# AndyCGraham/consensusClustR

Measured on AMD Instinct MI355X. Metric: bootstraps/sec (kNN+SNN+co-cluster) at 100k cells, 1/2/4/8 MI355X, higher is better.
Workload: dtype f64

## Files before the change

consensusclustr_amd/csrc/silhouette.hip:

```cpp
#include <math.h>
#include <stdlib.h>
#include <string.h>

#include <algorithm>
#include <vector>

#include "ccg_internal.h"

#define SIL_T 256
#define SIL_CGRP 4
#ifndef SIL_LG
#define SIL_LG 5
#endif

__host__ __device__ __forceinline__ int scale_exp(double bound) {
    if (!(bound > 0.0)) return 52;
    int e = 61 - (ilogb(bound) + 1);
    return e > 52 ? 52 : e;
}

struct SilSegs {
    int nseg;
    const int64_t* off;
    const int32_t* const* lab;
    const int* ts;
    const int* tw;
    double* const* mean;
    int32_t* const* ncl;
    int32_t* const* mns;
};
__device__ __forceinline__ int sil_seg_tile(const int* __restrict__ pre, int nseg, int b) {
    int lo = 0, hi = nseg - 1;
    while (lo < hi) {
        const int mid = (lo + hi + 1) >> 1;
        if (pre[mid] <= b) lo = mid;
        else hi = mid - 1;
    }
    return lo;
}
__device__ __forceinline__ int sil_seg_row(const int64_t* __restrict__ off, int nseg, int64_t r) {
    int lo = 0, hi = nseg - 1;
    while (lo < hi) {
        const int mid = (lo + hi + 1) >> 1;
        if (off[mid] <= r) lo = mid;
        else hi = mid - 1;
    }
    return lo;
}
__device__ __forceinline__ int sil_label(const int32_t* __restrict__ labels, int64_t m, const SilSegs& sg, int q,
                                         int l, int64_t r) {
    if (sg.nseg) {
        const int64_t o = sg.off[q];
        return sg.lab[q][(int64_t)l * (sg.off[q + 1] - o) + (r - o)];
    }
    return labels[(int64_t)l * m + r];
}

#define SIL_MAXABS_GRID 256
#define SIL_MAXABS_T 1024
__global__ __launch_bounds__(SIL_MAXABS_T) void sil_maxabs(const double* __restrict__ x, int64_t tot,
                                                           unsigned* __restrict__ bits) {
    __shared__ unsigned red[SIL_MAXABS_T / 64];
    double mx = 0.0, m1 = 0.0, m2 = 0.0, m3 = 0.0;
    const int64_t stp = (int64_t)gridDim.x * blockDim.x;
    int64_t t = (int64_t)blockIdx.x * blockDim.x + threadIdx.x;
    for (; t + 3 * stp < tot; t += 4 * stp) {
        mx = fmax(mx, fabs(x[t]));
        m1 = fmax(m1, fabs(x[t + stp]));
        m2 = fmax(m2, fabs(x[t + 2 * stp]));
        m3 = fmax(m3, fabs(x[t + 3 * stp]));
    }
    for (; t < tot; t += stp) mx = fmax(mx, fabs(x[t]));
    mx = fmax(fmax(mx, m1), fmax(m2, m3));
    unsigned local = __float_as_uint(nextafterf((float)mx, INFINITY));
    for (int o = 32; o > 0; o >>= 1) local = max(local, (unsigned)__shfl_xor((int)local, o, 64));
    if ((threadIdx.x & 63) == 0) red[threadIdx.x >> 6] = local;
    __syncthreads();
    if (threadIdx.x == 0) {
        unsigned b = red[0];
#pragma unroll
        for (int w = 1; w < SIL_MAXABS_T / 64; ++w) b = max(b, red[w]);
        atomicMax(bits, b);
    }
}

template <int DMAX>
__device__ __forceinline__ void load_row(const double* __restrict__ x, int64_t r, int d,
// ... 9 lines not shown
                                                      int L, int cmax,
                                                      const unsigned* __restrict__ maxabs_bits,
                                                      unsigned long long* __restrict__ gsum,
                                                      unsigned long long* __restrict__ gcnt) {
    extern __shared__ __attribute__((aligned(16))) unsigned char smem[];
    unsigned long long* acc = (unsigned long long*)smem;
    unsigned* cnt = (unsigned*)(acc + (int64_t)(cmax + 1) * d);
    const int64_t r = (int64_t)blockIdx.x * SIL_T + threadIdx.x;
    const bool in = r < m;
    const double maxabs = (double)__uint_as_float(*maxabs_bits);
    const double sc = ldexp(1.0, scale_exp(maxabs * (double)m));
    long long q[DMAX];
#pragma unroll
    for (int k = 0; k < DMAX; ++k) q[k] = (in && k < d) ? __double2ll_rn(x[r * d + k] * sc) : 0ll;
    const int nacc = (cmax + 1) * d;
    const int l1 = min(L, (int)(blockIdx.y + 1) * SIL_LG);
    for (int l = blockIdx.y * SIL_LG; l < l1; ++l) {
        unsigned long long* gs = gsum + (int64_t)l * nacc;
        unsigned long long* gc = gcnt + (int64_t)l * (cmax + 1);
        if (LDS) {
            for (int t = threadIdx.x; t < nacc; t += SIL_T) acc[t] = 0ull;
            for (int t = threadIdx.x; t <= cmax; t += SIL_T) cnt[t] = 0u;
            __syncthreads();
        }
        if (in) {
            const int lab = labels[(int64_t)l * m + r];
            if (lab >= 1 && lab <= cmax) {
#pragma unroll
                for (int k = 0; k < DMAX; ++k)
                    if (k < d) {
                        if (LDS) atomicAdd(&acc[lab * d + k], (unsigned long long)q[k]);
                        else atomicAdd(&gs[(int64_t)lab * d + k], (unsigned long long)q[k]);
                    }
                if (LDS) atomicAdd(&cnt[lab], 1u);
                else atomicAdd(&gc[lab], 1ull);
            }
        }
        if (LDS) {
            __syncthreads();
            for (int t = threadIdx.x; t < nacc; t += SIL_T)
                if (acc[t]) atomicAdd(&gs[t], acc[t]);
            for (int t = threadIdx.x; t <= cmax; t += SIL_T)
                if (cnt[t]) atomicAdd(&gc[t], (unsigned long long)cnt[t]);
            __syncthreads();
        }
    }
}

__device__ __forceinline__ int sil_block_excl_scan(int v, int* sh, int* total) {
    const int t = threadIdx.x, lane = t & 63, wv = t >> 6;
    int x = v;
    for (int o = 1; o < 64; o <<= 1) {
        const int y = __shfl_up(x, o, 64);
        if (lane >= o) x += y;
    }
    if (lane == 63) sh[wv] = x;
    __syncthreads();
    int woff = 0, tot = 0;
    for (int w = 0; w < SIL_T / 64; ++w) {
        if (w < wv) woff += sh[w];
        tot += sh[w];
    }
    __syncthreads();
    *total = tot;
    return woff + x - v;
}

__host__ __device__ inline double sil_s2_bound(double maxabs, int d, int64_t m) {
    return maxabs * maxabs * (double)d * (double)m;
}
template <int DMAX>
__global__ void sil_quant(const double* __restrict__ x, int64_t m, int d, const unsigned* __restrict__ maxabs_bits,
                          long long* __restrict__ q1, long long* __restrict__ q2) {
    const int64_t t = (int64_t)blockIdx.x * blockDim.x + threadIdx.x;
    const int64_t r = t / DMAX;
    if (r >= m) return;
    const int k = (int)(t - r * DMAX);
    const double maxabs = (double)__uint_as_float(*maxabs_bits);
    const double sc = ldexp(1.0, scale_exp(maxabs * (double)m));
    const double v = k < d ? x[r * d + k] : 0.0;
    const long long qv = __double2ll_rn(v * sc);
    q1[t] = qv;
    const double vq = (double)qv / sc;
    double s2 = vq * vq;
#pragma unroll
    for (int o = DMAX / 2; o > 0; o >>= 1) s2 += __shfl_xor(s2, o, 64);
    if (k == 0) q2[r] = __double2ll_rn(s2 * ldexp(1.0, scale_exp(sil_s2_bound(maxabs, d, m))));
}

#define SIL_SB 1024
#define SIL_SP 1024
#ifndef SIL_SGMAX
#define SIL_SGMAX 4
#endif
#define SIL_LDS_CU 163840
#ifndef SIL_LDS_SUMS
#define SIL_LDS_SUMS 81920
#endif
__host__ __device__ inline size_t sil_tile_lds(int d, int cmax, int G) {
    return (size_t)SIL_SP * 4 + (size_t)G * SIL_SP * 8 + (size_t)G * (cmax + 1) * (d + 2) * 8;
}
static inline int sil_sums_G(int d, int cmax) {
    for (int G = SIL_SGMAX; G >= 1; G >>= 1)
        if (sil_tile_lds(d, cmax, G) <= SIL_LDS_SUMS) return G;
    return sil_tile_lds(d, cmax, 1) <= SIL_LDS_CU ? 1 : 0;
}

template <int DMAX, bool SEG>
__global__ __launch_bounds__(SIL_SB) void sil_sums_blk(int64_t m, int d, int ntile, int tpx, int G,
                                                       const int32_t* __restrict__ labels, int L, int cmax,
                                                       const long long* __restrict__ q1,
                                                       const long long* __restrict__ q2,
                                                       unsigned long long* __restrict__ gsum,
                                                       unsigned long long* __restrict__ gsum2,
                                                       unsigned long long* __restrict__ gcnt,
                                                       const int* __restrict__ rep, const int* __restrict__ mult,
                                                       const int* __restrict__ cnt, int64_t mw,
                                                       const int64_t* __restrict__ nrep,
                                                       const int64_t* __restrict__ scan, SilSegs sgs) {
    extern __shared__ __attribute__((aligned(16))) unsigned char smem[];
    int* srow = (int*)smem;
    int* slab = srow + SIL_SP;
    int* swgt = slab + G * SIL_SP;
    unsigned long long* acc = (unsigned long long*)(swgt + G * SIL_SP);
    const int na = (cmax + 1) * (d + 2);
    constexpr int NW = SIL_SB / 64;
    constexpr int RPW = 64 / DMAX;
    constexpr int PPW = SIL_SP / NW;
    const int tid = threadIdx.x, lane = tid & 63, wave = tid >> 6;
    const int k = lane % DMAX, sub = lane / DMAX;
    const int loc = blockIdx.x >> 3;
    const int grp = loc / tpx;
    const int tile = (loc - grp * tpx) * 8 + (blockIdx.x & 7);
    const int l0 = grp * G;
    if (l0 >= L || tile >= ntile) return;
    const int ng = min(G, L - l0);
    int64_t rb, npos;
    int q = 0;
    if constexpr (SEG) {
        q = sil_seg_tile(sgs.ts, sgs.nseg, tile);
        rb = scan[sgs.off[q]] + (int64_t)(tile - sgs.ts[q]) * SIL_SP;
        npos = scan[sgs.off[q + 1]];
    } else {
        rb = (int64_t)tile * SIL_SP;
        npos = rep ? *nrep : m;
    }
    if (rb >= npos) return;
    for (int t = tid; t < ng * na; t += SIL_SB) acc[t] = 0ull;
    for (int p = tid; p < SIL_SP; p += SIL_SB) {
        const int64_t ps = rb + p;
        const bool in = ps < npos;
        const int row = in ? (rep ? rep[ps] : (int)ps) : 0;
        srow[p] = row;
        const int c0 = (in && rep) ? cnt[ps] : 1;
        for (int g = 0; g < G; ++g) {
            int lb = 0, wg = 0;
            if (in && g < ng) {
                const int l = l0 + g;
                if constexpr (SEG) lb = sil_label(labels, m, sgs, q, l, row);
                else lb = labels[(int64_t)l * m + row];
                wg = rep ? c0 - mult[(int64_t)l * mw + ps] : 1;
            }
            const bool ok = lb >= 1 && lb <= cmax && wg > 0;
            slab[g * SIL_SP + p] = ok ? lb : 0;
            swgt[g * SIL_SP + p] = ok ? wg : 0;
        }
    }
    __syncthreads();
    constexpr int SU = 8;
    static_assert((PPW / RPW) % SU == 0, "walk unroll");
    for (int i0 = 0; i0 < PPW / RPW; i0 += SU) {
        int rr[SU];
        long long v[SU], v2[SU];
#pragma unroll
        for (int u = 0; u < SU; ++u) rr[u] = srow[wave * PPW + (i0 + u) * RPW + sub];
#pragma unroll
        for (int u = 0; u < SU; ++u) {
            v[u] = q1[(int64_t)rr[u] * DMAX + k];
            v2[u] = q2[rr[u]];
        }
#pragma unroll
        for (int u = 0; u < SU; ++u) asm volatile("" : "+v"(v[u]), "+v"(v2[u]));
        for (int g = 0; g < ng; ++g) {
            unsigned long long* ag = acc + g * na;
#pragma unroll
            for (int u = 0; u < SU; ++u) {
                const int pl = g * SIL_SP + wave * PPW + (i0 + u) * RPW + sub;
                const int lb = slab[pl];
                if (lb) {
                    const long long w = swgt[pl];
                    if (k < d) atomicAdd(&ag[lb * d + k], (unsigned long long)(w * v[u]));
                    if (k == 0) {
                        atomicAdd(&ag[(cmax + 1) * d + lb], (unsigned long long)(w * v2[u]));
                        atomicAdd(&ag[(cmax + 1) * (d + 1) + lb], (unsigned long long)w);
                    }
                }
            }
        }
    }
    __syncthreads();
    for (int g = 0; g < ng; ++g) {
        const int lv = q * L + l0 + g;
        const unsigned long long* ag = acc + g * na;
        unsigned long long* gs = gsum + (int64_t)lv * (cmax + 1) * d;
        for (int t = tid; t < (cmax + 1) * d; t += SIL_SB) {
            const unsigned long long v = ag[t];
            if (v) atomicAdd(&gs[t], v);
        }
        for (int c = tid; c <= cmax; c += SIL_SB) {
            const unsigned long long n = ag[(cmax + 1) * (d + 1) + c];
            if (n) {
                atomicAdd(&gcnt[(int64_t)lv * (cmax + 1) + c], n);
                atomicAdd(&gsum2[(int64_t)lv * (cmax + 1) + c], ag[(cmax + 1) * d + c]);
            }
        }
    }
}

template <int DMAX>
__global__ void sil_sums_exc(int64_t m, int d, const int32_t* __restrict__ labels, int L, int cmax,
                             const long long* __restrict__ q1, const long long* __restrict__ q2,
                             const unsigned long long* __restrict__ exc, const int* __restrict__ nexc,
                             unsigned long long* __restrict__ gsum, unsigned long long* __restrict__ gsum2,
                             unsigned long long* __restrict__ gcnt, SilSegs sgs) {
    const int ne = *nexc;
    for (int e = blockIdx.x * blockDim.x + threadIdx.x; e < ne; e += gridDim.x * blockDim.x) {
        const int l = (int)(exc[e] >> 32);
        const int64_t r = (int64_t)(exc[e] & 0xffffffffull);
        const int q = sgs.nseg ? sil_seg_row(sgs.off, sgs.nseg, r) : 0;
        const int lab = sil_label(labels, m, sgs, q, l, r);
        if (lab < 1 || lab > cmax) continue;
        const int64_t lv = (int64_t)q * L + l;
        unsigned long long* gs = gsum + (lv * (cmax + 1) + lab) * d;
        for (int k = 0; k < d; ++k) atomicAdd(&gs[k], (unsigned long long)q1[r * DMAX + k]);
        atomicAdd(&gsum2[lv * (cmax + 1) + lab], (unsigned long long)q2[r]);
        atomicAdd(&gcnt[lv * (cmax + 1) + lab], 1ull);
    }
}

template <int DMAX>
__host__ __device__ __forceinline__ int sil_mfma_pos(int k) {
    constexpr int KS = DMAX / 4;
    return (k & 3) * KS + (k >> 2);
}

template <int DMAX>
__global__ __launch_bounds__(SIL_T) void sil_mu(int64_t m, int d, int cmax,
                                                const unsigned* __restrict__ maxabs_bits,
                                                const unsigned long long* __restrict__ gsum,
                                                const unsigned long long* __restrict__ gsum2,
                                                const unsigned long long* __restrict__ gcnt,
                                                int* __restrict__ npres, int* __restrict__ codes,
                                                int* __restrict__ pos, double* __restrict__ mu,
                                                double* __restrict__ muc, double* __restrict__ auxc) {
    __shared__ int sh[SIL_T / 64];
    const int l = blockIdx.x;
    const double maxabs = (double)__uint_as_float(*maxabs_bits);
    const double inv_sc = ldexp(1.0, -scale_exp(maxabs * (double)m));
    const unsigned long long* gs = gsum + (int64_t)l * (cmax + 1) * d;
    const unsigned long long* gc = gcnt + (int64_t)l * (cmax + 1);
    int* pl = pos + (int64_t)l * (cmax + 1);
    int carry = 0;
    for (int c0 = 0; c0 <= cmax; c0 += SIL_T) {
        const int c = c0 + threadIdx.x;
        const bool present = c >= 1 && c <= cmax && gc[c] != 0ull;
        int tot;
        const int ex = carry + sil_block_excl_scan(present ? 1 : 0, sh, &tot);
        if (c <= cmax) pl[c] = present ? ex : -1;
        if (present) codes[(int64_t)l * cmax + ex] = c;
        carry += tot;
    }
    if (threadIdx.x == 0) npres[l] = carry;
    __syncthreads();
    double* ml = mu + (int64_t)l * (cmax + 1) * DMAX;
    double* mcl = muc + (int64_t)l * cmax * DMAX;
    for (int64_t t = threadIdx.x; t < (int64_t)(cmax + 1) * DMAX; t += SIL_T) {
        const int c = (int)(t / DMAX), k = (int)(t - (int64_t)c * DMAX);
        const unsigned long long n = gc[c];
        const double v = (n && k < d) ? ((double)(long long)gs[(int64_t)c * d + k] * inv_sc) / (double)n : 0.0;
        ml[t] = v;
        const int pc = pl[c];
        if (pc >= 0) mcl[(int64_t)pc * DMAX + sil_mfma_pos<DMAX>(k)] = v;
    }
    __syncthreads();
    for (int c = threadIdx.x; c <= cmax; c += SIL_T) {
        const int pc = pl[c];
        if (pc < 0) continue;
        double s = 0.0;
        for (int k = 0; k < d; ++k) s = fma(ml[(int64_t)c * DMAX + k], ml[(int64_t)c * DMAX + k], s);
        auxc[((int64_t)l * cmax + pc) * 2] = s;
        if (gsum2) {
            const double inv_sc2 = ldexp(1.0, -scale_exp(sil_s2_bound(maxabs, d, m)));
            const double n = (double)gc[c];
            const double v = ((double)(long long)gsum2[(int64_t)l * (cmax + 1) + c] * inv_sc2) / n - s;
            const double floor_v = inv_sc2 + 0x1p-50 * s;
            auxc[((int64_t)l * cmax + pc) * 2 + 1] = v > floor_v ? v : 0.0;
        }
    }
}

template <int DMAX, bool LDS>
__global__ __launch_bounds__(SIL_T) void sil_var(const double* __restrict__ x, int64_t m, int d,
                                                 const int32_t* __restrict__ labels, int L, int cmax,
                                                 const unsigned* __restrict__ maxabs_bits,
                                                 const double* __restrict__ mu,
                                                 unsigned long long* __restrict__ gvar) {
    extern __shared__ __attribute__((aligned(16))) unsigned char smem[];
    double* mus = (double*)smem;
    unsigned long long* vacc = (unsigned long long*)(mus + (int64_t)(cmax + 1) * DMAX);
    const int64_t r = (int64_t)blockIdx.x * SIL_T + threadIdx.x;
    const bool in = r < m;
    double xr[DMAX];
    load_row<DMAX>(x, in ? r : 0, d, xr);
    const double maxabs = (double)__uint_as_float(*maxabs_bits);
    const double vb = 4.0 * maxabs * maxabs * (double)d * (double)m;
    const double vsc = ldexp(1.0, scale_exp(vb));
    const int l1 = min(L, (int)(blockIdx.y + 1) * SIL_LG);
    for (int l = blockIdx.y * SIL_LG; l < l1; ++l) {
        const double* ml = mu + (int64_t)l * (cmax + 1) * DMAX;
        unsigned long long* gv = gvar + (int64_t)l * (cmax + 1);
        if (LDS) {
            for (int t = threadIdx.x; t < (cmax + 1) * DMAX; t += SIL_T) mus[t] = ml[t];
// ... 722 lines not shown

#define SIL_MULT_LG 8
__global__ __launch_bounds__(256) void sil_mult_kernel(int64_t m, int L, const int32_t* __restrict__ labels,
                                                       const int64_t* __restrict__ scan,
                                                       const int3* __restrict__ nonrep, int64_t mw,
                                                       int* __restrict__ dis, unsigned long long* __restrict__ exc,
                                                       int* __restrict__ nexc, SilSegs sgs) {
    const int64_t nn = m - scan[m];
    for (int l0 = blockIdx.y * SIL_MULT_LG; l0 < L; l0 += gridDim.y * SIL_MULT_LG)
    for (int64_t j = (int64_t)blockIdx.x * blockDim.x + threadIdx.x; j < nn; j += (int64_t)gridDim.x * blockDim.x) {
        const int3 e = nonrep[j];
        const int r = e.x, rp = e.y;
        const int q = sgs.nseg ? sil_seg_row(sgs.off, sgs.nseg, r) : 0;
        int a[SIL_MULT_LG], b[SIL_MULT_LG];
#pragma unroll
        for (int t = 0; t < SIL_MULT_LG; ++t) {
            a[t] = b[t] = 0;
            if (l0 + t < L) {
                a[t] = sil_label(labels, m, sgs, q, l0 + t, r);
                b[t] = sil_label(labels, m, sgs, q, l0 + t, rp);
            }
        }
#pragma unroll
        for (int t = 0; t < SIL_MULT_LG; ++t) {
            if (a[t] != b[t]) {
                const int l = l0 + t;
                atomicAdd(&dis[(int64_t)l * mw + e.z], 1);
                const int x = atomicAdd(nexc, 1);
                exc[x] = ((unsigned long long)l << 32) | (unsigned long long)r;
            }
        }
    }
}

template <int DMAX>
__global__ void sil_width_exc(const double* __restrict__ x, int64_t m, int d, const int32_t* __restrict__ labels,
                              int L, int cmax, const int* __restrict__ npres, const int* __restrict__ codes,
                              const double* __restrict__ muc, const double* __restrict__ auxc,
                              const unsigned long long* __restrict__ exc, const int* __restrict__ nexc, int nbw,
                              unsigned long long* __restrict__ wsum, unsigned long long* __restrict__ wcnt,
                              SilSegs sgs) {
    const int ne = *nexc;
    for (int e = blockIdx.x * blockDim.x + threadIdx.x; e < ne; e += gridDim.x * blockDim.x) {
    const int l = (int)(exc[e] >> 32);
    const int64_t r = (int64_t)(exc[e] & 0xffffffffull);
    const int q = sgs.nseg ? sil_seg_row(sgs.off, sgs.nseg, r) : 0;
    const int lab = sil_label(labels, m, sgs, q, l, r);
    const int64_t lv = (int64_t)q * L + l;
    double xr[DMAX];
#pragma unroll
    for (int k = 0; k < DMAX; ++k) xr[k] = k < d ? x[r * d + k] : 0.0;
    const int np = npres[lv];
    double self = INFINITY, oth = INFINITY;
    for (int p = 0; p < np; ++p) {
        const double* mp = muc + (lv * cmax + p) * DMAX;
        double s2 = fmax(auxc[2 * (lv * cmax + p) + 1], 0.0);
#pragma unroll
        for (int k = 0; k < DMAX; ++k) {
            const double t = xr[k] - mp[sil_mfma_pos<DMAX>(k)];
            s2 = fma(t, t, s2);
        }
        if (codes[lv * cmax + p] == lab) self = s2;
        else oth = fmin(oth, s2);
    }
    long long wq = 0;
    unsigned wn = 0;
    sil_row_width(self, oth, true, np, ldexp(1.0, scale_exp((double)m)), nullptr, wq, wn);
    if (wn) {
        atomicAdd(&wsum[lv * nbw], (unsigned long long)wq);
        atomicAdd(&wcnt[lv * nbw], 1ull);
    }
    }
}

static int sil_tile_T(int d, int cmax) {
    return sil_sums_G(d, cmax) ? SIL_SP : 0;
}

template <int DMAX>
static void sil_launch(const double* x, int64_t m, int d, const int32_t* labels, int L, int cmax,
                       unsigned* maxabs, unsigned long long* gsum, unsigned long long* gsum2, unsigned long long* gcnt,
                       unsigned long long* gvar, unsigned long long* wsum, unsigned long long* wcnt,
                       int* npres, int* codes, int* pos, double* mu, double* muc, double* auxc, void* q,
                       unsigned char* img, double* out_width, int nbw, hipStream_t st, const int* rep = nullptr,
                       const int* mult = nullptr, const int* cnt = nullptr, int64_t mw = 0,
                       const unsigned long long* exc = nullptr, const int* nexc = nullptr,
                       const int64_t* nrep = nullptr, const int64_t* scan = nullptr, SilSegs sgs = SilSegs{},
                       int ts_tiles = 0, int tw_tiles = 0) {
    const bool seg = sgs.nseg > 0;
    const int Lv = seg ? sgs.nseg * L : L;
    const int T = q ? sil_tile_T(d, cmax) : 0;
    if (T) {
        long long* q1 = (long long*)q;
        long long* q2 = q1 + m * DMAX;
        sil_quant<DMAX><<<(unsigned)ccg_cdiv(m * DMAX, 256), 256, 0, st>>>(x, m, d, maxabs, q1, q2);
        const int ntile = (int)(seg ? ts_tiles : ccg_cdiv(m, T));
        const int tpx = (int)ccg_cdiv(ntile, 8);
        const int G = sil_sums_G(d, cmax);
        const unsigned gb = (unsigned)(8 * (int64_t)tpx * ccg_cdiv(L, G));
        const size_t lds = sil_tile_lds(d, cmax, G);
        if (seg)
            sil_sums_blk<DMAX, true><<<gb, SIL_SB, lds, st>>>(m, d, ntile, tpx, G, labels, L, cmax, q1, q2, gsum, gsum2,
                                                              gcnt, rep, mult, cnt, mw, nrep, scan, sgs);
        else
            sil_sums_blk<DMAX, false><<<gb, SIL_SB, lds, st>>>(m, d, ntile, tpx, G, labels, L, cmax, q1, q2, gsum, gsum2,
                                                               gcnt, rep, mult, cnt, mw, nrep, scan, sgs);
        if (rep)
            sil_sums_exc<DMAX><<<64, 256, 0, st>>>(m, d, labels, L, cmax, q1, q2, exc, nexc, gsum, gsum2, gcnt, sgs);
        sil_mu<DMAX><<<Lv, SIL_T, 0, st>>>(m, d, cmax, maxabs, gsum, gsum2, gcnt, npres, codes, pos, mu, muc, auxc);
    } else {
        dim3 grid((unsigned)ccg_cdiv(m, SIL_T), (unsigned)ccg_cdiv(L, SIL_LG));
        const size_t lds1 = (size_t)(cmax + 1) * d * 8 + (size_t)(cmax + 1) * 4;
        const size_t lds2 = (size_t)(cmax + 1) * DMAX * 8 + (size_t)(cmax + 1) * 8;
        if (lds1 <= SIL_LDS_CAP)
            sil_centroid<DMAX, true><<<grid, SIL_T, lds1, st>>>(x, m, d, labels, L, cmax, maxabs, gsum, gcnt);
        else
            sil_centroid<DMAX, false><<<grid, SIL_T, 0, st>>>(x, m, d, labels, L, cmax, maxabs, gsum, gcnt);
        sil_mu<DMAX><<<L, SIL_T, 0, st>>>(m, d, cmax, maxabs, gsum, nullptr, gcnt, npres, codes, pos, mu, muc, auxc);
        if (lds2 <= SIL_LDS_CAP)
            sil_var<DMAX, true><<<grid, SIL_T, lds2, st>>>(x, m, d, labels, L, cmax, maxabs, mu, gvar);
        else
            sil_var<DMAX, false><<<grid, SIL_T, 0, st>>>(x, m, d, labels, L, cmax, maxabs, mu, gvar);
        sil_vfin<<<(unsigned)ccg_cdiv((int64_t)L * (cmax + 1), 256), 256, 0, st>>>(m, d, L, cmax, maxabs, gcnt,
                                                                                    gvar, pos, auxc);
    }
    const int64_t nrows = rep ? mw : m;
    bool w16 = false;
    if constexpr (DMAX <= 32) w16 = cmax <= SIL_WCMAX && 2 * sil_img_stride(cmax, DMAX) <= SIL_W16_LDS && img;
    if (w16) {
        if constexpr (DMAX <= 32) {
        const size_t imgs = sil_img_stride(cmax, DMAX);
        sil_w16_prep<DMAX><<<Lv, 256, 0, st>>>(cmax, maxabs, npres, codes, pos, mu, auxc, img, imgs);
        dim3 g16((unsigned)(seg ? tw_tiles : ccg_cdiv(nrows, SIL_WT / 2)), (unsigned)ccg_cdiv(L, SIL_WLG));
        const double wsc = ldexp(1.0, scale_exp((double)m)), sqd = sqrt((double)d);
        double* ow = rep ? nullptr : out_width;
#define SIL_W16(B_)                                                                                                  \
        if (seg)                                                                                                     \
            sil_width16<DMAX, B_, true><<<g16, SIL_WT, 0, st>>>(x, m, d, labels, L, cmax, maxabs, npres, img, imgs,  \
                                                                wsum, wcnt, ow, rep, mult, cnt, mw, nbw, nrep, wsc,  \
                                                                sqd, scan, sgs);                                     \
        else                                                                                                         \
            sil_width16<DMAX, B_, false><<<g16, SIL_WT, 0, st>>>(x, m, d, labels, L, cmax, maxabs, npres, img, imgs, \
                                                                 wsum, wcnt, ow, rep, mult, cnt, mw, nbw, nrep, wsc, \
                                                                 sqd, scan, sgs)
        if (imgs <= 14336) { SIL_W16(14336); }
        else if (imgs <= 26624) { SIL_W16(26624); }
        else { SIL_W16(40960); }
#undef SIL_W16
        if (rep)
            sil_width_exc<DMAX><<<64, 256, 0, st>>>(x, m, d, labels, L, cmax, npres, codes, muc, auxc, exc, nexc, nbw,
                                                    wsum, wcnt, sgs);
        }
        return;
    }
    dim3 grid2((unsigned)ccg_cdiv(nrows, sil_width_rows<DMAX>()), (unsigned)ccg_cdiv(L, SIL_LG));
    const int CH = (int)std::min<int64_t>(sil_chunk<DMAX>(), (int64_t)SIL_LG * (((int64_t)cmax + 15) / 16 * 16));
    const size_t lds5 = (size_t)CH * sil_sp<DMAX>() * 8 + (size_t)CH * 8 + (size_t)CH * 4;
    if (rep) {
        sil_width<DMAX><<<grid2, SIL_T, lds5, st>>>(x, m, d, labels, L, cmax, npres, codes, muc, auxc, wsum, wcnt,
                                                nullptr, CH, rep, mult, cnt, mw, nbw, nrep);
        sil_width_exc<DMAX><<<64, 256, 0, st>>>(x, m, d, labels, L, cmax, npres, codes, muc, auxc, exc, nexc, nbw,
                                                wsum, wcnt, sgs);
    } else {
        sil_width<DMAX><<<grid2, SIL_T, lds5, st>>>(x, m, d, labels, L, cmax, npres, codes, muc, auxc, wsum, wcnt,
                                                out_width, CH, nullptr, nullptr, nullptr, 0, nbw, nullptr);
    }
}

extern "C" int ccg_silhouette_dev(ccg_ctx* ctx, const double* x, int64_t m, int d,
                                  const int32_t* labels, int L, int cmax, double* out_mean,
                                  int32_t* out_nclust, int32_t* out_minsize, double* out_width,
                                  void* stream) {
    CCG_REQUIRE(ctx && x && labels, "ccg_silhouette_dev: NULL argument");
    CCG_REQUIRE(m >= 1 && m < (1LL << 31) && d >= 1 && d <= 64 && L >= 1,
                "ccg_silhouette_dev: bad sizes m=%lld d=%d L=%d", (long long)m, d, L);
    CCG_REQUIRE(cmax >= 1 && cmax <= (1 << 24), "ccg_silhouette_dev: cmax=%d must be in [1, 2^24]", cmax);
    hipStream_t st = ccg_pick_stream(ctx, stream);
    const int64_t nacc = (int64_t)(cmax + 1) * d;
    const int nbw = sil_width_blocks(m, d);
    const int64_t words = 2 * (int64_t)L * nacc + 2 * (int64_t)L * (cmax + 1) + 2 * (int64_t)L * nbw + 8;
    unsigned long long* buf = (unsigned long long*)ccg_ws(ctx, WS_SIL_A, sizeof(unsigned long long) * words);
    if (!buf) return CCG_ENOMEM;
    unsigned long long* gsum = buf;
    unsigned long long* gsum2 = gsum + (int64_t)L * nacc;
    unsigned long long* gcnt = gsum2 + (int64_t)L * nacc;
    unsigned long long* gvar = gcnt + (int64_t)L * (cmax + 1);
    unsigned long long* wsum = gvar + (int64_t)L * (cmax + 1);
    unsigned long long* wcnt = wsum + (int64_t)L * nbw;
    unsigned* maxabs = (unsigned*)(wcnt + (int64_t)L * nbw);
    const int dmax = d <= 16 ? 16 : (d <= 32 ? 32 : 64);
    const size_t mu_words = (size_t)L * (cmax + 1) * dmax + (size_t)L * cmax * dmax + 2 * (size_t)L * cmax;
    const size_t tab_ints = (size_t)L * cmax + (size_t)L * (cmax + 1) + L + 8;
    double* mu = (double*)ccg_ws(ctx, WS_SIL_B, sizeof(double) * mu_words + sizeof(int) * tab_ints);
    if (!mu) return CCG_ENOMEM;
    double* muc = mu + (size_t)L * (cmax + 1) * dmax;
    double* auxc = muc + (size_t)L * cmax * dmax;
    int* npres = (int*)(auxc + 2 * (size_t)L * cmax);
    int* codes = npres + L;
    int* pos = codes + (size_t)L * cmax;
    void* q = nullptr;
    if (sil_tile_T(d, cmax)) {
        q = ccg_ws(ctx, WS_SIL_Q, sizeof(long long) * (size_t)m * dmax + sizeof(long long) * (size_t)m + 64);
        if (!q) return CCG_ENOMEM;
    }
    unsigned char* img = nullptr;
    if (dmax <= 32 && cmax <= SIL_WCMAX && 2 * sil_img_stride(cmax, dmax) <= SIL_W16_LDS) {
        img = (unsigned char*)ccg_ws(ctx, WS_SIL_IMG, (size_t)L * sil_img_stride(cmax, dmax));
        if (!img) return CCG_ENOMEM;
    }
    const int t_all = ccg_timer_start(ctx, CCG_KT_SILHOUETTE, st);
    CCG_HIP(hipMemsetAsync(buf, 0, sizeof(unsigned long long) * words, st));
    sil_maxabs<<<(unsigned)std::min<int64_t>(ccg_cdiv(m * d, 4 * SIL_MAXABS_T), SIL_MAXABS_GRID), SIL_MAXABS_T, 0,
                 st>>>(x, m * d, maxabs);
    if (d <= 16)
        sil_launch<16>(x, m, d, labels, L, cmax, maxabs, gsum, gsum2, gcnt, gvar, wsum, wcnt, npres, codes, pos, mu, muc, auxc, q,
                        img, out_width, nbw, st);
    else if (d <= 32)
        sil_launch<32>(x, m, d, labels, L, cmax, maxabs, gsum, gsum2, gcnt, gvar, wsum, wcnt, npres, codes, pos, mu, muc, auxc, q,
                        img, out_width, nbw, st);
    else
        sil_launch<64>(x, m, d, labels, L, cmax, maxabs, gsum, gsum2, gcnt, gvar, wsum, wcnt, npres, codes, pos, mu, muc, auxc, q,
                        img, out_width, nbw, st);
    sil_final<<<L, 256, 0, st>>>(m, L, cmax, nbw, gcnt, wsum, wcnt, out_mean, out_nclust, out_minsize, SilSegs{});
    ccg_timer_stop(ctx, t_all, st);
    CCG_HIP(hipGetLastError());
    return CCG_OK;
}

static int sil_cells_run(ccg_ctx* ctx, const double* x, int64_t m, int d, const int32_t* labels, int L, int cmax,
                         const int32_t* cell, int64_t ncell, double* out_mean, int32_t* out_nclust,
                         int32_t* out_minsize, hipStream_t st, SilSegs sgs, int ts_tiles, int tw_tiles, int nbw) {
    const int64_t Lv = sgs.nseg ? (int64_t)sgs.nseg * L : L;
    const int64_t nacc = (int64_t)(cmax + 1) * d;
    const int64_t words = 2 * Lv * nacc + 2 * Lv * (cmax + 1) + 2 * Lv * nbw + 8;
    unsigned long long* buf = (unsigned long long*)ccg_ws(ctx, WS_SIL_A, sizeof(unsigned long long) * words);
    if (!buf) return CCG_ENOMEM;
    unsigned long long* gsum = buf;
    unsigned long long* gsum2 = gsum + Lv * nacc;
    unsigned long long* gcnt = gsum2 + Lv * nacc;
    unsigned long long* gvar = gcnt + Lv * (cmax + 1);
    unsigned long long* wsum = gvar + Lv * (cmax + 1);
    unsigned long long* wcnt = wsum + Lv * nbw;
    unsigned* maxabs = (unsigned*)(wcnt + Lv * nbw);
    const int dmax = d <= 16 ? 16 : (d <= 32 ? 32 : 64);
    const size_t mu_words = (size_t)Lv * (cmax + 1) * dmax + (size_t)Lv * cmax * dmax + 2 * (size_t)Lv * cmax;
    const size_t tab_ints = (size_t)Lv * cmax + (size_t)Lv * (cmax + 1) + Lv + 8;
    double* mu = (double*)ccg_ws(ctx, WS_SIL_B, sizeof(double) * mu_words + sizeof(int) * tab_ints);
    if (!mu) return CCG_ENOMEM;
    double* muc = mu + (size_t)Lv * (cmax + 1) * dmax;
    double* auxc = muc + (size_t)Lv * cmax * dmax;
    int* npres = (int*)(auxc + 2 * (size_t)Lv * cmax);
    int* codes = npres + Lv;
    int* pos = codes + (size_t)Lv * cmax;
    void* q = nullptr;
    if (sil_tile_T(d, cmax)) {
        q = ccg_ws(ctx, WS_SIL_Q, sizeof(long long) * (size_t)m * dmax + sizeof(long long) * (size_t)m + 64);
        if (!q) return CCG_ENOMEM;
    }
    unsigned char* img = nullptr;
    if (dmax <= 32 && cmax <= SIL_WCMAX && 2 * sil_img_stride(cmax, dmax) <= SIL_W16_LDS) {
        img = (unsigned char*)ccg_ws(ctx, WS_SIL_IMG, (size_t)Lv * sil_img_stride(cmax, dmax));
        if (!img) return CCG_ENOMEM;
    }
    char* tb = (char*)ccg_ws(ctx, WS_SIL_C, sizeof(int) * (size_t)ncell + sizeof(int64_t) * (size_t)(m + 1) +
                                                5 * sizeof(int) * (size_t)m + sizeof(int) * (size_t)L * m +
                                                sizeof(unsigned long long) * (size_t)L * m + 512);
    if (!tb) return CCG_ENOMEM;
    int* first = (int*)tb;
    int64_t* scan = (int64_t*)(tb + ccg_cdiv(sizeof(int) * ncell, 16) * 16);
    int* rep = (int*)(scan + m + 1);
    int3* nonrep = (int3*)(rep + m);
    int* nexc = (int*)(nonrep + m);
    int* cnt = nexc + 4;
    int* mult = cnt + m;
    unsigned long long* exc =
        (unsigned long long*)(tb + ccg_cdiv((int64_t)((char*)(mult + (int64_t)L * m) - tb), 16) * 16);
    const int t_all = ccg_timer_start(ctx, CCG_KT_SILHOUETTE, st);
    const unsigned gm = (unsigned)ccg_cdiv(m, 256);
    sil_init_kernel<<<(unsigned)std::min<int64_t>(
                          ccg_cdiv(std::max(std::max(ncell, (int64_t)(L + 1) * m + 4), words), 256), 4096),
                      256, 0, st>>>(first, ncell, nexc, (int64_t)(L + 1) * m + 4, buf, words);
    sil_first_kernel<<<gm, 256, 0, st>>>(cell, m, first);
    sil_isrep_kernel<<<gm, 256, 0, st>>>(cell, m, first, scan);
    int rc = ccg_scan_i64(ctx, scan, scan, m, st);
    if (rc) return rc;
    sil_rep_kernel<<<gm, 256, 0, st>>>(cell, m, first, scan, rep, cnt, nonrep);
    dim3 gx((unsigned)ccg_cdiv(m, 512), (unsigned)std::min<int64_t>(ccg_cdiv(L, SIL_MULT_LG), 65535));
    sil_mult_kernel<<<gx, 256, 0, st>>>(m, L, labels, scan, nonrep, m, mult, exc, nexc, sgs);
    sil_maxabs<<<(unsigned)std::min<int64_t>(ccg_cdiv(m * d, 4 * SIL_MAXABS_T), SIL_MAXABS_GRID), SIL_MAXABS_T, 0,
                 st>>>(x, m * d, maxabs);
#define SIL_CELLS(DM_)                                                                                              \
    sil_launch<DM_>(x, m, d, labels, L, cmax, maxabs, gsum, gsum2, gcnt, gvar, wsum, wcnt, npres, codes, pos, mu, muc, \
                    auxc, q, img, nullptr, nbw, st, rep, mult, cnt, m, exc, nexc, scan + m, scan, sgs, ts_tiles,     \
                    tw_tiles)
    if (d <= 16) SIL_CELLS(16);
    else if (d <= 32) SIL_CELLS(32);
    else SIL_CELLS(64);
#undef SIL_CELLS
    sil_final<<<(unsigned)Lv, 256, 0, st>>>(m, L, cmax, nbw, gcnt, wsum, wcnt, out_mean, out_nclust, out_minsize, sgs);
    ccg_timer_stop(ctx, t_all, st);
    CCG_HIP(hipGetLastError());
    return CCG_OK;
}

extern "C" int ccg_silhouette_cells_dev(ccg_ctx* ctx, const double* x, int64_t m, int d, const int32_t* labels,
                                        int L, int cmax, const int32_t* cell, int64_t ncell, double* out_mean,
                                        int32_t* out_nclust, int32_t* out_minsize, void* stream) {
    CCG_REQUIRE(ctx && x && labels && cell, "ccg_silhouette_cells_dev: NULL argument");
    CCG_REQUIRE(m >= 1 && m < (1LL << 31) && d >= 1 && d <= 64 && L >= 1 && (int64_t)L * m < (1LL << 31),
                "ccg_silhouette_cells_dev: bad sizes m=%lld d=%d L=%d", (long long)m, d, L);
    CCG_REQUIRE(cmax >= 1 && cmax <= (1 << 24), "ccg_silhouette_cells_dev: cmax=%d must be in [1, 2^24]", cmax);
    CCG_REQUIRE(ncell >= 1 && ncell < (1LL << 31), "ccg_silhouette_cells_dev: bad ncell");
    hipStream_t st = ccg_pick_stream(ctx, stream);
    return sil_cells_run(ctx, x, m, d, labels, L, cmax, cell, ncell, out_mean, out_nclust, out_minsize, st, SilSegs{},
                         0, 0, sil_width_blocks(m, d));
}

extern "C" int ccg_silhouette_segments_dev(ccg_ctx* ctx, const double* x, int d, int nseg, const int64_t* seg_off,
                                           const int32_t* const* labels, int L, int cmax, const int32_t* cell,
                                           int64_t ncell, double* const* out_mean, int32_t* const* out_nclust,
                                           int32_t* const* out_minsize, void* stream) {
    CCG_REQUIRE(ctx && x && seg_off && labels && cell, "ccg_silhouette_segments_dev: NULL argument");
    CCG_REQUIRE(nseg >= 1 && d >= 1 && d <= 64 && L >= 1, "ccg_silhouette_segments_dev: bad sizes nseg=%d d=%d L=%d",
                nseg, d, L);
    CCG_REQUIRE(cmax >= 1 && cmax <= (1 << 24), "ccg_silhouette_segments_dev: cmax=%d must be in [1, 2^24]", cmax);
    CCG_REQUIRE(ncell >= 1 && ncell < (1LL << 31), "ccg_silhouette_segments_dev: bad ncell");
    CCG_REQUIRE(seg_off[0] == 0, "ccg_silhouette_segments_dev: seg_off[0] must be 0");
    int64_t mq_max = 0;
    for (int s = 0; s < nseg; ++s) {
        CCG_REQUIRE(seg_off[s + 1] > seg_off[s], "ccg_silhouette_segments_dev: segment %d is empty", s);
        CCG_REQUIRE(labels[s], "ccg_silhouette_segments_dev: labels of segment %d are NULL", s);
        mq_max = std::max(mq_max, seg_off[s + 1] - seg_off[s]);
    }
    const int64_t m = seg_off[nseg];
    CCG_REQUIRE(m < (1LL << 31) && (int64_t)L * m < (1LL << 31) && (int64_t)nseg * L < (1LL << 31),
                "ccg_silhouette_segments_dev: %lld rows x %d labelings too many", (long long)m, L);
    hipStream_t st = ccg_pick_stream(ctx, stream);
    const int dmax = d <= 16 ? 16 : (d <= 32 ? 32 : 64);
    const int T = sil_tile_T(d, cmax);
    const bool one_set = dmax <= 32 && T && cmax <= SIL_WCMAX && 2 * sil_img_stride(cmax, dmax) <= SIL_W16_LDS;
    if (!one_set) {
        for (int s = 0; s < nseg; ++s) {
            const int64_t o = seg_off[s];
            const int rc = ccg_silhouette_cells_dev(ctx, x + o * d, seg_off[s + 1] - o, d, labels[s], L, cmax, cell + o,
                                                    ncell, out_mean ? out_mean[s] : nullptr,
                                                    out_nclust ? out_nclust[s] : nullptr,
                                                    out_minsize ? out_minsize[s] : nullptr, st);
            if (rc) return rc;
        }
        return CCG_OK;
    }
    const size_t n1 = (size_t)nseg + 1;
    const size_t bytes = 8 * n1 + 8 * n1 + 8 * (size_t)nseg * 4;
    std::vector<unsigned char> hb(bytes);
    int64_t* hoff = (int64_t*)hb.data();
    int* hts = (int*)(hoff + n1);
    int* htw = hts + n1;
    const void** hptr = (const void**)(hts + 2 * n1 + ((2 * n1) & 1));
    int64_t ts = 0, tw = 0;
    for (size_t s = 0; s < n1; ++s) {
        hoff[s] = seg_off[s];
        hts[s] = (int)ts;
        htw[s] = (int)tw;
        if (s < (size_t)nseg) {
            const int64_t mq = seg_off[s + 1] - seg_off[s];
            ts += ccg_cdiv(mq, T);
            tw += ccg_cdiv(mq, SIL_WT / 2);
        }
    }
    CCG_REQUIRE(ts < (1LL << 31) && tw < (1LL << 31), "ccg_silhouette_segments_dev: too many tiles");
    for (int s = 0; s < nseg; ++s) {
        hptr[s] = labels[s];
        hptr[nseg + s] = out_mean ? out_mean[s] : nullptr;
        hptr[2 * nseg + s] = out_nclust ? out_nclust[s] : nullptr;
        hptr[3 * nseg + s] = out_minsize ? out_minsize[s] : nullptr;
    }
// ... 85 lines not shown
```

Measured before the change: 1199.

## Compute silhouette per-cluster sums with int8 MFMA on byte-split quantized rows

Adds a new sums kernel that quantizes each row inside the block and splits the 64-bit fixed-point values into signed 8-bit limbs staged in LDS. Per-cluster sums, squared norms and counts are then computed as int8 MFMA products of one-hot label/weight matrices against the limbs, and the limbs are recombined before atomics. Rows with large weights and exception rows fall back to per-row atomic adds. This replaces the separate quantize pass and the scatter/tile sums path when d<=32 and cmax<=255, which is meant to remove global q1/q2 traffic and scalar accumulation. The cost is more complex exactness-sensitive code. It is the default path, with an environment variable to go back to scatter.

```diff
diff --git a/consensusclustr_amd/csrc/silhouette.hip b/consensusclustr_amd/csrc/silhouette.hip
--- a/consensusclustr_amd/csrc/silhouette.hip
+++ b/consensusclustr_amd/csrc/silhouette.hip
@@ -3,6 +3,7 @@
 #include <string.h>
 
 #include <algorithm>
+#include <type_traits>
 #include <vector>
 
 #include "ccg_internal.h"
@@ -178,9 +179,10 @@
     const long long qv = __double2ll_rn(v * sc);
     q1[t] = qv;
     const double vq = (double)qv / sc;
-    double s2 = vq * vq;
-#pragma unroll
-    for (int o = DMAX / 2; o > 0; o >>= 1) s2 += __shfl_xor(s2, o, 64);
+    const double sq = vq * vq;
+    double s2 = fma(vq, vq, __shfl_xor(sq, DMAX / 2, 64));
+#pragma unroll
+    for (int o = DMAX / 4; o > 0; o >>= 1) s2 += __shfl_xor(s2, o, 64);
     if (k == 0) q2[r] = __double2ll_rn(s2 * ldexp(1.0, scale_exp(sil_s2_bound(maxabs, d, m))));
 }
 
@@ -334,6 +336,263 @@
     }
 }
 
+#define SIL_MT 512
+#define SIL_MB 512
+#define SIL_MSTR (SIL_MT + 16)
+#define SIL_MCMAX 255
+typedef int sil_v4i __attribute__((ext_vector_type(4)));
+typedef int sil_v16i __attribute__((ext_vector_type(16)));
+static_assert(SIL_SP % SIL_MT == 0, "a segment's sums tiles split into whole MFMA tiles");
+static_assert(SIL_MT == SIL_MB, "one position per thread while staging");
+
+__host__ __device__ inline size_t sil_mfma_lds(int NL) {
+    return (size_t)NL * 32 * SIL_MSTR + 2 * SIL_MT * sizeof(int) + (SIL_MB / 64) * 2 * SIL_MT + 16;
+}
+static inline int sil_mfma_limbs(int64_t m) {
+    int lg = 0;
+    while ((m >> (lg + 1)) > 0) ++lg;
+    return (61 - lg + 2 + 7) / 8;
+}
+
+template <int DMAX>
+__device__ __forceinline__ long long sil_quant_row(const double* __restrict__ xr, int d, double sc, double inv_sc,
+                                                   double sc2, long long (&q)[DMAX]) {
+#pragma clang fp contract(off)
+    double vq[DMAX], s[DMAX / 2];
+#pragma unroll
+    for (int k = 0; k < DMAX; ++k) {
+        q[k] = k < d ? __double2ll_rn(xr[k] * sc) : 0ll;
+        vq[k] = (double)q[k] * inv_sc;
+    }
+#pragma unroll
+    for (int k = 0; k < DMAX / 2; ++k) s[k] = fma(vq[k], vq[k], vq[k + DMAX / 2] * vq[k + DMAX / 2]);
+#pragma unroll
+    for (int o = DMAX / 4; o > 0; o >>= 1)
+#pragma unroll
+        for (int k = 0; k < o; ++k) s[k] = s[k] + s[k + o];
+    return __double2ll_rn(s[0] * sc2);
+}
+
+template <int DMAX>
+__device__ __noinline__ void sil_add_row(const double* __restrict__ x, int64_t r, int d, int64_t m, double maxabs,
+                                         long long w, unsigned long long* __restrict__ gs,
+                                         unsigned long long* __restrict__ g2, unsigned long long* __restrict__ gc) {
+    const int e = scale_exp(maxabs * (double)m);
+    long long q[DMAX];
+    const long long q2 = sil_quant_row<DMAX>(x + r * d, d, ldexp(1.0, e), ldexp(1.0, -e),
+                                             ldexp(1.0, scale_exp(sil_s2_bound(maxabs, d, m))), q);
+#pragma unroll
+    for (int k = 0; k < DMAX; ++k)
+        if (k < d) atomicAdd(&gs[k], (unsigned long long)(w * q[k]));
+    atomicAdd(g2, (unsigned long long)(w * q2));
+    atomicAdd(gc, (unsigned long long)w);
+}
+
+template <int DMAX, int NL, bool SEG>
+__global__ __launch_bounds__(SIL_MB) void sil_sums_mfma(const double* __restrict__ x, int64_t m, int d,
+                                                        const int32_t* __restrict__ labels, int L, int cmax,
+                                                        const unsigned* __restrict__ maxabs_bits,
+                                                        unsigned long long* __restrict__ gsum,
+                                                        unsigned long long* __restrict__ gsum2,
+                                                        unsigned long long* __restrict__ gcnt,
+                                                        const int* __restrict__ rep, const int* __restrict__ mult,
+                                                        const int* __restrict__ cnt, int64_t mw,
+                                                        const int64_t* __restrict__ nrep,
+                                                        const int64_t* __restrict__ scan, SilSegs sgs) {
+    static_assert(DMAX <= 32, "at most two column tiles");
+    extern __shared__ __attribute__((aligned(16))) unsigned char smem[];
+    unsigned char* bq = smem;
+    int* srow = (int*)(smem + (size_t)NL * 32 * SIL_MSTR);
+    int* scnt = srow + SIL_MT;
+    unsigned char* swl = (unsigned char*)(scnt + SIL_MT);
+    int* snext = (int*)(swl + (SIL_MB / 64) * 2 * SIL_MT);
+    constexpr int NCT = (DMAX + 2 + 31) / 32;
+    const int tid = threadIdx.x, lane = tid & 63, wave = tid >> 6, h = lane >> 5;
+    int64_t rb, npos;
+    int q = 0;
+    if constexpr (SEG) {
+        constexpr int SUB = SIL_SP / SIL_MT;
+        const int tile = blockIdx.x / SUB;
+        q = sil_seg_tile(sgs.ts, sgs.nseg, tile);
+        rb = scan[sgs.off[q]] + (int64_t)(tile - sgs.ts[q]) * SIL_SP + (int64_t)(blockIdx.x % SUB) * SIL_MT;
+        npos = scan[sgs.off[q + 1]];
+    } else {
+        rb = (int64_t)blockIdx.x * SIL_MT;
+        npos = rep ? *nrep : m;
+    }
+    if (rb >= npos) return;
+    const int nval = (int)min((int64_t)SIL_MT, npos - rb);
+    const double maxabs = (double)__uint_as_float(*maxabs_bits);
+    const bool valid = tid < nval;
+    const int myrow = valid ? (rep ? rep[rb + tid] : (int)(rb + tid)) : 0;
+    srow[tid] = myrow;
+    scnt[tid] = (valid && rep) ? cnt[rb + tid] : 1;
+    if (tid < 2) snext[tid] = 0;
+    long long qr[DMAX];
+    long long q2 = 0;
+    if (valid) {
+        const int e = scale_exp(maxabs * (double)m);
+        q2 = sil_quant_row<DMAX>(x + (int64_t)myrow * d, d, ldexp(1.0, e), ldexp(1.0, -e),
+                                 ldexp(1.0, scale_exp(sil_s2_bound(maxabs, d, m))), qr);
+    } else {
+#pragma unroll
+        for (int k = 0; k < DMAX; ++k) qr[k] = 0;
+    }
+    unsigned char* wl = swl + wave * 2 * SIL_MT;
+    unsigned char* ww = wl + SIL_MT;
+    const int nks = (nval + 31) >> 5;
+    auto pass = [&](auto CT) {
+        constexpr int ct = decltype(CT)::value;
+#pragma unroll
+        for (int c = 0; c < 32; ++c) {
+            const int col = ct * 32 + c;
+            if (col >= DMAX + 2 || col >= d + 2) continue;
+            long long v = 0;
+            if (col < DMAX) v = qr[col < DMAX ? col : 0];
+            if (col == d) v = q2;
+            if (col == d + 1) v = valid ? 1 : 0;
+#pragma unroll
+            for (int j = 0; j < NL; ++j) {
+                const signed char dj = (signed char)(v & 0xff);
+                bq[((size_t)j * 32 + c) * SIL_MSTR + tid] = (unsigned char)dj;
+                v = (v - dj) >> 8;
+            }
+        }
+        __syncthreads();
+        for (;;) {
+            int l = 0;
+            if (lane == 0) l = atomicAdd(&snext[ct], 1);
+            l = blockIdx.y + gridDim.y * __builtin_amdgcn_readfirstlane(l);
+            if (l >= L) break;
+            const int64_t lv = (int64_t)q * L + l;
+            constexpr int NP = SIL_MT / 256;
+            int lbv[NP][4], wgv[NP][4], rwv[NP][4];
+#pragma unroll
+            for (int hh = 0; hh < NP; ++hh) {
+                const int p0 = hh * 256 + lane * 4;
+                const int4 rw = *reinterpret_cast<const int4*>(&srow[p0]);
+                const int4 cw = *reinterpret_cast<const int4*>(&scnt[p0]);
+                const int rws[4] = {rw.x, rw.y, rw.z, rw.w}, cws[4] = {cw.x, cw.y, cw.z, cw.w};
+#pragma unroll
+                for (int i = 0; i < 4; ++i) {
+                    lbv[hh][i] = 0;
+                    wgv[hh][i] = 0;
+                    rwv[hh][i] = rws[i];
+                    if (p0 + i < nval) {
+                        if constexpr (SEG) lbv[hh][i] = sil_label(labels, m, sgs, q, l, rws[i]);
+                        else lbv[hh][i] = labels[(int64_t)l * m + rws[i]];
+                        wgv[hh][i] = rep ? cws[i] - mult[(int64_t)l * mw + rb + p0 + i] : 1;
+                    }
+                }
+            }
+            int mx = 0;
+#pragma unroll
+            for (int hh = 0; hh < NP; ++hh) {
+                const int p0 = hh * 256 + lane * 4;
+                unsigned lpk = 0, wpk = 0;
+#pragma unroll
+                for (int i = 0; i < 4; ++i) {
+                    const int lb = lbv[hh][i], wg = wgv[hh][i];
+                    bool ok = lb >= 1 && lb <= cmax && wg > 0;
+                    if (ok && wg > 127) {
+                        if (ct == 0)
+                            sil_add_row<DMAX>(x, rwv[hh][i], d, m, maxabs, wg,
+                                              gsum + (lv * (cmax + 1) + lb) * d, gsum2 + lv * (cmax + 1) + lb,
+                                              gcnt + lv * (cmax + 1) + lb);
+                        ok = false;
+                    }
+                    if (ok) {
+                        lpk |= (unsigned)lb << (8 * i);
+                        wpk |= (unsigned)wg << (8 * i);
+                        mx = max(mx, lb);
+                    }
+                }
+                *reinterpret_cast<unsigned*>(&wl[p0]) = lpk;
+                *reinterpret_cast<unsigned*>(&ww[p0]) = wpk;
+            }
+            for (int o = 32; o > 0; o >>= 1) mx = max(mx, __shfl_xor(mx, o, 64));
+            __builtin_amdgcn_wave_barrier();
+            asm volatile("" ::: "memory");
+            const int nblk = mx ? (mx >> 5) + 1 : 0;
+            for (int cb = 0; cb < nblk; ++cb) {
+                sil_v16i acc[NL];
+#pragma unroll
+                for (int j = 0; j < NL; ++j)
+#pragma unroll
+                    for (int r = 0; r < 16; ++r) acc[j][r] = 0;
+                const unsigned i4 = (unsigned)(cb * 32 + (lane & 31)) * 0x01010101u;
+                const unsigned char* bl = bq + (size_t)(lane & 31) * SIL_MSTR + h * 16;
+                for (int ks = 0; ks < nks; ++ks) {
+                    const int kb = ks * 32 + h * 16;
+                    const sil_v4i l4 = *reinterpret_cast<const sil_v4i*>(wl + kb);
+                    const sil_v4i w4 = *reinterpret_cast<const sil_v4i*>(ww + kb);
+                    sil_v4i a;
+#pragma unroll
+                    for (int t = 0; t < 4; ++t) {
+                        const unsigned xo = (unsigned)l4[t] ^ i4;
+                        const unsigned nz = ((xo & 0x7f7f7f7fu) + 0x7f7f7f7fu) | xo;
+                        const unsigned eq = (~nz & 0x80808080u) >> 7;
+                        a[t] = (int)((unsigned)w4[t] & (eq * 0xffu));
+                    }
+#pragma unroll
+                    for (int j = 0; j < NL; ++j) {
+                        const sil_v4i b = *reinterpret_cast<const sil_v4i*>(bl + (size_t)j * 32 * SIL_MSTR + ks * 32);
+                        acc[j] = __builtin_amdgcn_mfma_i32_32x32x32_i8(a, b, acc[j], 0, 0, 0);
+                    }
+                }
+                const int col = ct * 32 + (lane & 31);
+#pragma unroll
+                for (int r = 0; r < 16; ++r) {
+                    const int c = cb * 32 + (r & 3) + 8 * (r >> 2) + 4 * h;
+                    unsigned long long s = 0;
+#pragma unroll
+                    for (int j = 0; j < NL; ++j) s += (unsigned long long)(long long)acc[j][r] << (8 * j);
+                    if (s && c <= cmax && col < d + 2) {
+                        const int64_t lc = lv * (cmax + 1) + c;
+                        if (col < d) atomicAdd(&gsum[lc * d + col], s);
+                        else if (col == d) atomicAdd(&gsum2[lc], s);
+                        else atomicAdd(&gcnt[lc], s);
+                    }
+                }
+            }
+            __builtin_amdgcn_wave_barrier();
+            asm volatile("" ::: "memory");
+        }
+    };
+    pass(std::integral_constant<int, 0>{});
+    if constexpr (NCT > 1) {
+        if (d + 2 > 32) {
+            __syncthreads();
+            pass(std::integral_constant<int, 1>{});
+        }
+    }
+}
+
+template <int DMAX>
+__global__ void sil_sums_exc_x(const double* __restrict__ x, int64_t m, int d, const int32_t* __restrict__ labels,
+                               int L, int cmax, const unsigned* __restrict__ maxabs_bits,
+                               const unsigned long long* __restrict__ exc, const int* __restrict__ nexc,
+                               unsigned long long* __restrict__ gsum, unsigned long long* __restrict__ gsum2,
+                               unsigned long long* __restrict__ gcnt, SilSegs sgs) {
+    const int ne = *nexc;
+    const double maxabs = (double)__uint_as_float(*maxabs_bits);
+    for (int e = blockIdx.x * blockDim.x + threadIdx.x; e < ne; e += gridDim.x * blockDim.x) {
+        const int l = (int)(exc[e] >> 32);
+        const int64_t r = (int64_t)(exc[e] & 0xffffffffull);
+        const int q = sgs.nseg ? sil_seg_row(sgs.off, sgs.nseg, r) : 0;
+        const int lab = sil_label(labels, m, sgs, q, l, r);
+        if (lab < 1 || lab > cmax) continue;
+        const int64_t lc = ((int64_t)q * L + l) * (cmax + 1) + lab;
+        sil_add_row<DMAX>(x, r, d, m, maxabs, 1, gsum + lc * d, gsum2 + lc, gcnt + lc);
+    }
+}
+
+static bool sil_use_mfma(int d, int cmax) {
+    if (d > 32 || cmax > SIL_MCMAX) return false;
+    const char* p = getenv("CCG_SIL_SUMS");
+    return !(p && !strcmp(p, "scatter"));
+}
+
 template <int DMAX>
 __host__ __device__ __forceinline__ int sil_mfma_pos(int k) {
     constexpr int KS = DMAX / 4;
@@ -1222,7 +1481,7 @@
                        unsigned* maxabs, unsigned long long* gsum, unsigned long long* gsum2, unsigned long long* gcnt,
                        unsigned long long* gvar, unsigned long long* wsum, unsigned long long* wcnt,
                        int* npres, int* codes, int* pos, double* mu, double* muc, double* auxc, void* q,
-                       unsigned char* img, double* out_width, int nbw, hipStream_t st, const int* rep = nullptr,
+                       bool mfma, unsigned char* img, double* out_width, int nbw, hipStream_t st, const int* rep = nullptr,
                        const int* mult = nullptr, const int* cnt = nullptr, int64_t mw = 0,
                        const unsigned long long* exc = nullptr, const int* nexc = nullptr,
                        const int64_t* nrep = nullptr, const int64_t* scan = nullptr, SilSegs sgs = SilSegs{},
@@ -1230,7 +1489,26 @@
     const bool seg = sgs.nseg > 0;
     const int Lv = seg ? sgs.nseg * L : L;
     const int T = q ? sil_tile_T(d, cmax) : 0;
-    if (T) {
+    if (mfma) {
+        if constexpr (DMAX <= 32) {
+            const unsigned gt = (unsigned)(seg ? (int64_t)ts_tiles * (SIL_SP / SIL_MT) : ccg_cdiv(m, SIL_MT));
+            const dim3 gb(gt, (unsigned)std::max(1, std::min(std::min(8, L), (int)(512 / gt))));
+#define SIL_MF(NL_)                                                                                                  \
+            if (seg)                                                                                                 \
+                sil_sums_mfma<DMAX, NL_, true><<<gb, SIL_MB, sil_mfma_lds(NL_), st>>>(                               \
+                    x, m, d, labels, L, cmax, maxabs, gsum, gsum2, gcnt, rep, mult, cnt, mw, nrep, scan, sgs);       \
+            else                                                                                                     \
+                sil_sums_mfma<DMAX, NL_, false><<<gb, SIL_MB, sil_mfma_lds(NL_), st>>>(                              \
+                    x, m, d, labels, L, cmax, maxabs, gsum, gsum2, gcnt, rep, mult, cnt, mw, nrep, scan, sgs)
+            if (sil_mfma_limbs(m) <= 6) { SIL_MF(6); }
+            else { SIL_MF(8); }
+#undef SIL_MF
+            if (rep)
+                sil_sums_exc_x<DMAX><<<64, 256, 0, st>>>(x, m, d, labels, L, cmax, maxabs, exc, nexc, gsum, gsum2,
+                                                         gcnt, sgs);
+            sil_mu<DMAX><<<Lv, SIL_T, 0, st>>>(m, d, cmax, maxabs, gsum, gsum2, gcnt, npres, codes, pos, mu, muc, auxc);
+        }
+    } else if (T) {
         long long* q1 = (long long*)q;
         long long* q2 = q1 + m * DMAX;
         sil_quant<DMAX><<<(unsigned)ccg_cdiv(m * DMAX, 256), 256, 0, st>>>(x, m, d, maxabs, q1, q2);
@@ -1338,8 +1616,9 @@
     int* npres = (int*)(auxc + 2 * (size_t)L * cmax);
     int* codes = npres + L;
     int* pos = codes + (size_t)L * cmax;
+    const bool mfma = sil_use_mfma(d, cmax);
     void* q = nullptr;
-    if (sil_tile_T(d, cmax)) {
+    if (!mfma && sil_tile_T(d, cmax)) {
         q = ccg_ws(ctx, WS_SIL_Q, sizeof(long long) * (size_t)m * dmax + sizeof(long long) * (size_t)m + 64);
         if (!q) return CCG_ENOMEM;
     }
@@ -1354,13 +1633,13 @@
                  st>>>(x, m * d, maxabs);
     if (d <= 16)
         sil_launch<16>(x, m, d, labels, L, cmax, maxabs, gsum, gsum2, gcnt, gvar, wsum, wcnt, npres, codes, pos, mu, muc, auxc, q,
-                        img, out_width, nbw, st);
+                        mfma, img, out_width, nbw, st);
     else if (d <= 32)
         sil_launch<32>(x, m, d, labels, L, cmax, maxabs, gsum, gsum2, gcnt, gvar, wsum, wcnt, npres, codes, pos, mu, muc, auxc, q,
-                        img, out_width, nbw, st);
+                        mfma, img, out_width, nbw, st);
     else
         sil_launch<64>(x, m, d, labels, L, cmax, maxabs, gsum, gsum2, gcnt, gvar, wsum, wcnt, npres, codes, pos, mu, muc, auxc, q,
-                        img, out_width, nbw, st);
+                        mfma, img, out_width, nbw, st);
     sil_final<<<L, 256, 0, st>>>(m, L, cmax, nbw, gcnt, wsum, wcnt, out_mean, out_nclust, out_minsize, SilSegs{});
     ccg_timer_stop(ctx, t_all, st);
     CCG_HIP(hipGetLastError());
@@ -1392,8 +1671,9 @@
     int* npres = (int*)(auxc + 2 * (size_t)Lv * cmax);
     int* codes = npres + Lv;
     int* pos = codes + (size_t)Lv * cmax;
+    const bool mfma = sil_use_mfma(d, cmax);
     void* q = nullptr;
-    if (sil_tile_T(d, cmax)) {
+    if (!mfma && sil_tile_T(d, cmax)) {
         q = ccg_ws(ctx, WS_SIL_Q, sizeof(long long) * (size_t)m * dmax + sizeof(long long) * (size_t)m + 64);
         if (!q) return CCG_ENOMEM;
     }
@@ -1431,7 +1711,7 @@
                  st>>>(x, m * d, maxabs);
 #define SIL_CELLS(DM_)                                                                                              \
     sil_launch<DM_>(x, m, d, labels, L, cmax, maxabs, gsum, gsum2, gcnt, gvar, wsum, wcnt, npres, codes, pos, mu, muc, \
-                    auxc, q, img, nullptr, nbw, st, rep, mult, cnt, m, exc, nexc, scan + m, scan, sgs, ts_tiles,     \
+                    auxc, q, mfma, img, nullptr, nbw, st, rep, mult, cnt, m, exc, nexc, scan + m, scan, sgs, ts_tiles,     \
                     tw_tiles)
     if (d <= 16) SIL_CELLS(16);
     else if (d <= 32) SIL_CELLS(32);
```

Measured after the change: 1267, median of 6. 1.06x the previous value.
